# yunjinli/visual-slam

Hardware: AMD Instinct MI355X
Metric: stereo frames/sec, detect+describe (1500 feats) + stereo match, 752x480 (higher is better)
Workload: dtype u8/f32/f64; 1 GPU; synthetic 752x480 stereo, 1500 feats/frame (BASELINE configs[1]); independent streams per GPU (configs[3]); inputs_resident_in_hbm=True, distinct_stereo_pairs_per_gpu=1024, distinct_scenes_per_gpu=64, stereo_frames_per_pass_per_gpu=1024, hip_streams=2, stereo_frames_per_launch=512, num_features=1500, match=threshold 70, ratio 1.2, cross-check

## Files before the change

### visual-slam_amd/csrc/match.hip

```cpp
#include "vsl_common.h"

#ifndef VSL_MATCH_WAVES
#define VSL_MATCH_WAVES 8
#endif
#define KEY_SHIFT 22
#define KEY_INIT ((256u << KEY_SHIFT) | 0u)

__device__ __forceinline__ uint32_t umed3(uint32_t a, uint32_t b, uint32_t c) {
  uint32_t r;
  asm("v_med3_u32 %0, %1, %2, %3" : "=v"(r) : "v"(a), "v"(b), "v"(c));
  return r;
}

template <int WAVES>
__global__ __launch_bounds__(64 * WAVES) void hamming_best2_kernel(
    const uint64_t* __restrict__ desc, const int32_t* __restrict__ kp_count,
    const int32_t* __restrict__ pair_slots, uint32_t* __restrict__ best_key,
    uint32_t* __restrict__ second_key, int F) {
  const int pair = blockIdx.z, dir = blockIdx.y;
  const int slot_r = pair_slots[2 * pair + dir];
  const int slot_c = pair_slots[2 * pair + 1 - dir];
  const int n_r = kp_count[slot_r], n_c = kp_count[slot_c];
  const int row0 = blockIdx.x * 64;
  if (row0 >= n_r) return;
  const int lane = threadIdx.x & 63;
  const int wave = __builtin_amdgcn_readfirstlane(threadIdx.x >> 6);
  const int row = row0 + lane;

  uint32_t r[8];
  {
    const uint32_t* p = (const uint32_t*)(desc + ((size_t)slot_r * F + (row < n_r ? row : 0)) * 4);
#pragma unroll
    for (int k = 0; k < 8; k++) r[k] = p[k];
  }
  int chunk = (n_c + WAVES - 1) / WAVES;
  chunk = (chunk + 3) & ~3;
  const int c0 = wave * chunk;
  const int c1 = min(n_c, c0 + chunk);
  const uint32_t* __restrict__ cbase = (const uint32_t*)(desc + (size_t)slot_c * F * 4);

  uint32_t b = KEY_INIT, s = KEY_INIT;
  int j = c0;
  for (; j + 4 <= c1; j += 4) {
#pragma unroll
    for (int u = 0; u < 4; u++) {
      const uint32_t* __restrict__ c = cbase + (size_t)(j + u) * 8;
      uint32_t d = 0;
#pragma unroll
      for (int k = 0; k < 8; k++) d += __builtin_popcount(r[k] ^ c[k]);
      const uint32_t key = (d << KEY_SHIFT) | (uint32_t)(j + u);
      s = umed3(b, key, s);
      b = min(b, key);
    }
  }
  for (; j < c1; j++) {
    const uint32_t* __restrict__ c = cbase + (size_t)j * 8;
    uint32_t d = 0;
#pragma unroll
    for (int k = 0; k < 8; k++) d += __builtin_popcount(r[k] ^ c[k]);
    const uint32_t key = (d << KEY_SHIFT) | (uint32_t)j;
    s = umed3(b, key, s);
    b = min(b, key);
  }

  __shared__ uint32_t sb[WAVES][64], ss[WAVES][64];
  sb[wave][lane] = b;
  ss[wave][lane] = s;
  __syncthreads();
  if (wave == 0 && row < n_r) {
#pragma unroll
    for (int w = 1; w < WAVES; w++) {
      const uint32_t b2 = sb[w][lane], s2 = ss[w][lane];
      s = min(umed3(b, b2, s), s2);
      b = min(b, b2);
    }
    const size_t o = ((size_t)pair * 2 + dir) * F + row;
    best_key[o] = b;
    second_key[o] = s;
  }
}

typedef int v4i_t __attribute__((ext_vector_type(4)));
typedef int v16i_t __attribute__((ext_vector_type(16)));

#define MM_PAD_KEY (1023u << KEY_SHIFT)
#define MM_ROW 272

__device__ __forceinline__ v4i_t expand16(uint32_t bits16) {
  v4i_t o;
  o.x = (int)((((bits16 >> 0) & 15u) * 0x00204081u) & 0x01010101u);
  o.y = (int)((((bits16 >> 4) & 15u) * 0x00204081u) & 0x01010101u);
  o.z = (int)((((bits16 >> 8) & 15u) * 0x00204081u) & 0x01010101u);
  o.w = (int)((((bits16 >> 12) & 15u) * 0x00204081u) & 0x01010101u);
  return o;
}

#ifndef MM_WAVES
#define MM_WAVES 8
#endif
template <bool STAGGER>
__global__ __launch_bounds__(64 * MM_WAVES) void hamming_mfma_kernel(const uint64_t* __restrict__ desc,
                                                           const int32_t* __restrict__ kp_count,
                                                           const int32_t* __restrict__ pair_slots,
                                                           uint32_t* __restrict__ best_key,
                                                           uint32_t* __restrict__ second_key, int F) {
  __shared__ __align__(16) unsigned char tile[2][64 * MM_ROW];
  __shared__ __align__(16) uint32_t rowkey[3][64];
  const int pair = blockIdx.z, dir = blockIdx.y;
  const int slot_q = pair_slots[2 * pair + dir];
  const int slot_d = pair_slots[2 * pair + 1 - dir];
  const int n_q = kp_count[slot_q], n_d = kp_count[slot_d];
  const int q0 = blockIdx.x * (32 * MM_WAVES);
  if (q0 >= n_q) return;
  const int tid = threadIdx.x, lane = tid & 63, wave = tid >> 6;
  const int c = lane & 31, h = lane >> 5;
  const int qc = q0 + wave * 32 + c;
  const uint32_t* __restrict__ qd = (const uint32_t*)(desc + ((size_t)slot_q * F + (qc < n_q ? qc : 0)) * 4);
  const uint32_t* __restrict__ dbase = (const uint32_t*)(desc + (size_t)slot_d * F * 4);

  v4i_t bq[8];
  int pq = 0;
#pragma unroll
  for (int s = 0; s < 8; s++) {
    const uint32_t wq = qd[s];
    pq += __builtin_popcount(wq);
    const v4i_t e = expand16((wq >> (16 * h)) & 0xFFFFu);
    bq[s].x = (int)((uint32_t)e.x * 0xFEu + 0x01010101u);
    bq[s].y = (int)((uint32_t)e.y * 0xFEu + 0x01010101u);
    bq[s].z = (int)((uint32_t)e.z * 0xFEu + 0x01010101u);
    bq[s].w = (int)((uint32_t)e.w * 0xFEu + 0x01010101u);
  }

  constexpr int FILL_K = 64 * MM_WAVES >= 512 ? 1 : 512 / (64 * MM_WAVES);
  const bool filler = tid < 512;
  constexpr int FILL_ROWS = 64 / FILL_K;
  const int frow = tid >> 3, fword = tid & 7;
  auto load_words = [&](int st, uint32_t& w0, uint32_t& w1) {
    const int r0 = st * 64 + frow, r1 = r0 + FILL_ROWS;
    w0 = (filler && r0 < n_d) ? dbase[(size_t)r0 * 8 + fword] : 0u;
    w1 = (FILL_K > 1 && r1 < n_d) ? dbase[(size_t)r1 * 8 + fword] : 0u;
  };
  auto store_rows = [&](int buf, int st, uint32_t w0, uint32_t w1) {
    if (!filler) return;
#pragma unroll
    for (int k = 0; k < FILL_K; k++) {
      const uint32_t wd = k ? w1 : w0;
      const int lr = frow + FILL_ROWS * k;
      unsigned char* dst = &tile[buf][lr * MM_ROW + fword * 32];
      *(v4i_t*)dst = expand16(wd & 0xFFFFu);
      *(v4i_t*)(dst + 16) = expand16(wd >> 16);
      const int m = st * 64 + lr;
      if (fword == 0) rowkey[st % 3][lr] = m < n_d ? ((256u << KEY_SHIFT) | (uint32_t)m) : MM_PAD_KEY;
    }
  };
  const int n_st = (n_d + 63) / 64;
  uint32_t b = 0xFFFFFFFFu, sk = 0xFFFFFFFFu, bB = 0xFFFFFFFFu, skB = 0xFFFFFFFFu;
  {
    uint32_t w0, w1;
    load_words(0, w0, w1);
    store_rows(0, 0, w0, w1);
    __syncthreads();
  }
  v16i_t acc0, acc1;
  auto mfma_phase = [&](int buf) {
    acc0 = (v16i_t){0, 0, 0, 0, 0, 0, 0, 0, 0, 0, 0, 0, 0, 0, 0, 0};
    acc1 = (v16i_t){0, 0, 0, 0, 0, 0, 0, 0, 0, 0, 0, 0, 0, 0, 0, 0};
#pragma unroll
    for (int s = 0; s < 8; s++) {
      const v4i_t a0 = *(const v4i_t*)&tile[buf][c * MM_ROW + s * 32 + h * 16];
      const v4i_t a1 = *(const v4i_t*)&tile[buf][(c + 32) * MM_ROW + s * 32 + h * 16];
      acc0 = __builtin_amdgcn_mfma_i32_32x32x32_i8(a0, bq[s], acc0, 0, 0, 0);
      acc1 = __builtin_amdgcn_mfma_i32_32x32x32_i8(a1, bq[s], acc1, 0, 0, 0);
    }
  };
  auto key_phase = [&](int rk_slot) {
#pragma unroll
    for (int half = 0; half < 2; half++) {
#pragma unroll
      for (int g = 0; g < 4; g++) {
        const uint4 rk = *(const uint4*)&rowkey[rk_slot][32 * half + 8 * g + 4 * h];
        const uint32_t rks[4] = {rk.x, rk.y, rk.z, rk.w};
#pragma unroll
        for (int j = 0; j < 4; j++) {
          const int av = half ? acc1[4 * g + j] : acc0[4 * g + j];
          const uint32_t key = ((uint32_t)av << KEY_SHIFT) + rks[j];
          if (half) {
            skB = umed3(bB, key, skB);
            bB = min(bB, key);
          } else {
            sk = umed3(b, key, sk);
            b = min(b, key);
          }
        }
      }
    }
  };
  const bool late = STAGGER && wave >= MM_WAVES / 2;
  for (int st = 0; st < n_st; st++) {
    const int buf = st & 1;
    uint32_t n0 = 0, n1 = 0;
    if (st + 1 < n_st) load_words(st + 1, n0, n1);
    if (late) {
      if (st > 0) key_phase((st - 1) % 3);
      mfma_phase(buf);
    } else {
      mfma_phase(buf);
      key_phase(st % 3);
    }
    if (st + 1 < n_st) store_rows(buf ^ 1, st + 1, n0, n1);
    __syncthreads();
  }
  if (late && n_st > 0) key_phase((n_st - 1) % 3);
  sk = min(umed3(b, bB, sk), skB);
  b = min(b, bB);
  const uint32_t b2 = (uint32_t)__shfl_xor((int)b, 32), s2 = (uint32_t)__shfl_xor((int)sk, 32);
  sk = min(umed3(b, b2, sk), s2);
  b = min(b, b2);
  if (h == 0 && qc < n_q) {
    const uint32_t fix = (uint32_t)(pq - 256) << KEY_SHIFT;
    const size_t o = ((size_t)pair * 2 + dir) * F + qc;
    best_key[o] = (b >> KEY_SHIFT) >= 1023u ? KEY_INIT : b + fix;
    second_key[o] = (sk >> KEY_SHIFT) >= 1023u ? KEY_INIT : sk + fix;
  }
}

typedef int v8i_t __attribute__((ext_vector_type(8)));
typedef float v16f_t __attribute__((ext_vector_type(16)));
#define MX_ROW 144
#define MX_KEY_SCALE 2048.0f
#define MX_KEY_BIAS 512.0f
#define MX_PAD_KEY_F 4096.0f

__global__ __launch_bounds__(512) void match_select_kernel(const int32_t* __restrict__ kp_count, const int32_t* __restrict__ pair_slots,
                                                           const uint32_t* __restrict__ best_key,
                                                           const uint32_t* __restrict__ second_key, int F, int threshold,
                                                           double dist_2_best, int32_t* __restrict__ sel_list,
                                                           int32_t* __restrict__ sel_count) {
  __shared__ unsigned char flag[2048];
  __shared__ int sel_wave[8];
  const int pair = blockIdx.x, tid = threadIdx.x, lane = tid & 63, wave = tid >> 6;
  const int n_a = kp_count[pair_slots[2 * pair]], n_b = kp_count[pair_slots[2 * pair + 1]];
  const uint32_t* bk0 = best_key + ((size_t)pair * 2) * F;
  const uint32_t* sk0 = second_key + ((size_t)pair * 2) * F;
  for (int j = tid; j < 2048; j += 512) flag[j] = 0;
  __syncthreads();
  for (int i = tid; i < n_a; i += 512) {
    const uint32_t bk = bk0[i];
    const int d1 = (int)(bk >> KEY_SHIFT), d2 = (int)(sk0[i] >> KEY_SHIFT);
    if (n_b > 0 && d1 < threshold && !((double)d2 < (double)d1 * dist_2_best)) flag[bk & ((1u << KEY_SHIFT) - 1)] = 1;
  }
  __syncthreads();
  int cnt = 0;
#pragma unroll
  for (int u = 0; u < 4; u++) cnt += flag[tid * 4 + u];
  int incl = cnt;
#pragma unroll
  for (int d = 1; d < 64; d <<= 1) {
    const int o = __shfl_up(incl, d);
    if (lane >= d) incl += o;
  }
  if (lane == 63) sel_wave[wave] = incl;
  __syncthreads();
  int base = 0, total = 0;
#pragma unroll
  for (int w = 0; w < 8; w++) {
    if (w < wave) base += sel_wave[w];
    total += sel_wave[w];
  }
  int pos = base + incl - cnt;
  int32_t* out = sel_list + (size_t)pair * 2 * F;
#pragma unroll
  for (int u = 0; u < 4; u++)
    if (flag[tid * 4 + u]) out[pos++] = tid * 4 + u;
  if (tid == 0) sel_count[pair] = total;
}

#ifndef MX_WAVES_PER_EU
#define MX_WAVES_PER_EU 6
#endif
#ifndef MX_TIMING
#define MX_TIMING 0
#endif
#define MX_OCC __attribute__((amdgpu_waves_per_eu(MX_WAVES_PER_EU, MX_WAVES_PER_EU)))
#if MX_TIMING
__device__ long long mx_dbg[4 * 16];
__device__ long long mx_tl[4 * 3072];
extern "C" int vsl_mx_timing(long long* out) { return (int)hipMemcpyFromSymbol(out, HIP_SYMBOL(mx_dbg), sizeof(mx_dbg)); }
extern "C" int vsl_mx_timeline(long long* out) { return (int)hipMemcpyFromSymbol(out, HIP_SYMBOL(mx_tl), sizeof(mx_tl)); }
#endif
template <bool REVERSE>
__global__ __launch_bounds__(64 * MM_WAVES) MX_OCC void hamming_mx_kernel(const uint64_t* __restrict__ desc,
                                                                   const int32_t* __restrict__ kp_count,
                                                                   const int32_t* __restrict__ pair_slots,
                                                                   uint32_t* __restrict__ best_key,
                                                                   uint32_t* __restrict__ second_key, int F, int n_pairs,
                                                                   int blocks_per_pair, const int32_t* __restrict__ sel_list,
                                                                   const int32_t* __restrict__ sel_count, int both_dirs) {
  __shared__ __align__(16) unsigned char tile[2][64 * MX_ROW];
  __shared__ __align__(16) float rowkey[64];
  __shared__ uint32_t lut[256];
#if MX_TIMING
  const long long wEntry = wall_clock64();
#endif
  const int xj = (int)(blockIdx.x >> 3);
  const int pair = (xj / blocks_per_pair) * 8 + (int)(blockIdx.x & 7u);
  if (pair >= n_pairs) return;
  int blk = xj % blocks_per_pair;
  int dir = REVERSE ? 1 : 0;
  if (!REVERSE && both_dirs) {
    const int half = blocks_per_pair >> 1;
    dir = blk >= half ? 1 : 0;
    blk -= dir * half;
  }
  const int slot_q = pair_slots[2 * pair + dir];
  const int slot_d = pair_slots[2 * pair + 1 - dir];
  int n_q = kp_count[slot_q];
  const int n_d = kp_count[slot_d];
  const int q0 = blk * (32 * MM_WAVES);
  const int tid = threadIdx.x, lane = tid & 63, wave = tid >> 6;
  const int c = lane & 31, h = lane >> 5;
  const int32_t* __restrict__ sel = sel_list + (size_t)pair * 2 * F;
  if (REVERSE) n_q = sel_count[pair];
  if (q0 >= n_q) return;
  const int qc = q0 + wave * 32 + c;
  const int qrow = REVERSE ? sel[qc < n_q ? qc : 0] : (qc < n_q ? qc : 0);
  const uint32_t* __restrict__ qd = (const uint32_t*)(desc + ((size_t)slot_q * F + qrow) * 4);
  const uint32_t* __restrict__ dbase = (const uint32_t*)(desc + (size_t)slot_d * F * 4);
  if (tid < 256) {
    uint32_t x = (uint32_t)tid;
    x = (x | (x << 12)) & 0x000F000Fu;
    x = (x | (x << 6)) & 0x03030303u;
    x = (x | (x << 3)) & 0x11111111u;
    lut[tid] = x << 1;
  }
  __syncthreads();
  auto spread = [&](uint32_t w) -> v4i_t {
    v4i_t o;
    o.x = (int)lut[w & 255u];
    o.y = (int)lut[(w >> 8) & 255u];
    o.z = (int)lut[(w >> 16) & 255u];
    o.w = (int)lut[w >> 24];
    return o;
  };
  auto fp4_operand = [](v4i_t t) -> v8i_t { return __builtin_shufflevector(t, t, 0, 1, 2, 3, -1, -1, -1, -1); };
  v8i_t bq[4];
  int pq = 0;
#pragma unroll
  for (int s = 0; s < 4; s++) {
    const uint32_t w0 = qd[2 * s], w1 = qd[2 * s + 1];
    pq += __builtin_popcount(w0) + __builtin_popcount(w1);
    const v4i_t e = spread(h ? w1 : w0);
    bq[s] = fp4_operand((v4i_t){(int)(((uint32_t)e.x << 2) | 0x22222222u), (int)(((uint32_t)e.y << 2) | 0x22222222u),
                                (int)(((uint32_t)e.z << 2) | 0x22222222u), (int)(((uint32_t)e.w << 2) | 0x22222222u)});
  }
  const bool filler = tid < 512;
  const int frow = tid >> 3, fword = tid & 7;
  const int n_st = (n_d + 63) / 64;
  auto load_word = [&](int st) -> uint32_t {
    const int r0 = st * 64 + frow;
    return (filler && r0 < n_d) ? dbase[(size_t)r0 * 8 + fword] : 0u;
  };
  auto store_row = [&](int buf, int st, uint32_t wd) {
    if (!filler) return;
    *(v4i_t*)&tile[buf][frow * MX_ROW + fword * 16] = spread(wd);
    const int m = st * 64 + frow;
    if (fword == 0 && st == n_st - 1) rowkey[frow] = m < n_d ? (MX_KEY_BIAS + (float)m * (1.0f / MX_KEY_SCALE)) : MX_PAD_KEY_F;
  };
  uint32_t b = 0xFFFFFFFFu, sk = 0xFFFFFFFFu;
  auto fold3 = [](uint32_t& B, uint32_t& S, uint32_t k1, uint32_t k2, uint32_t k3) {
    const uint32_t lo = min(min(k1, k2), k3), mid = umed3(k1, k2, k3);
    S = umed3(B, lo, min(S, mid));
    B = min(B, lo);
  };
  auto tile_best2 = [&](uint32_t& L, uint32_t& M, const v16f_t& a) {
    uint32_t lo[5], mid[5];
#pragma unroll
    for (int t = 0; t < 5; t++) {
      const uint32_t k1 = __float_as_uint(a[3 * t]), k2 = __float_as_uint(a[3 * t + 1]), k3 = __float_as_uint(a[3 * t + 2]);
      lo[t] = min(min(k1, k2), k3);
      mid[t] = __float_as_uint(__builtin_amdgcn_fmed3f(a[3 * t], a[3 * t + 1], a[3 * t + 2]));
    }
    L = min(min(lo[0], lo[1]), lo[2]);
    M = umed3(lo[0], lo[1], lo[2]);
    fold3(L, M, lo[3], lo[4], __float_as_uint(a[15]));
    M = min(M, min(min(min(mid[0], mid[1]), mid[2]), min(mid[3], mid[4])));
  };
  v16f_t start;
#pragma unroll
  for (int i = 0; i < 16; i++) start[i] = MX_KEY_BIAS + (float)(8 * (i >> 2) + 4 * h + (i & 3)) * (1.0f / MX_KEY_SCALE);
  store_row(0, 0, load_word(0));
  __syncthreads();
  float tile_first = 0.0f;
  const bool idle = __builtin_amdgcn_readfirstlane(q0 + wave * 32) >= n_q;
#if MX_TIMING
  long long tA = 0, tB = 0, tC = 0;
  const long long w0 = wall_clock64();
#endif
  for (int st = 0; st < n_st; st++) {
#if MX_TIMING
    const long long s0 = __builtin_amdgcn_s_memtime();
#endif
    const int buf = st & 1;
    uint32_t nw = 0;
    if (st + 1 < n_st) nw = load_word(st + 1);
#define MX_QUAD(half, s) fp4_operand(*(const v4i_t*)&tile[buf][(c + 32 * (half)) * MX_ROW + (s) * 32 + h * 16])
    if (!idle)
#pragma unroll
    for (int half = 0; half < 2; half++) {
      v16f_t acc;
      if (st + 1 < n_st) {
        acc = __builtin_amdgcn_mfma_scale_f32_32x32x64_f8f6f4(MX_QUAD(half, 0), bq[0], start, 4, 4, 0, 127, 0, 127);
      } else {
#pragma unroll
        for (int g = 0; g < 4; g++) {
          const float4 r = *(const float4*)&rowkey[32 * half + 8 * g + 4 * h];
          acc[4 * g] = r.x, acc[4 * g + 1] = r.y, acc[4 * g + 2] = r.z, acc[4 * g + 3] = r.w;
        }
        acc = __builtin_amdgcn_mfma_scale_f32_32x32x64_f8f6f4(MX_QUAD(half, 0), bq[0], acc, 4, 4, 0, 127, 0, 127);
      }
#pragma unroll
      for (int s = 1; s < 4; s++) acc = __builtin_amdgcn_mfma_scale_f32_32x32x64_f8f6f4(MX_QUAD(half, s), bq[s], acc, 4, 4, 0, 127, 0, 127);
      uint32_t l, m;
      tile_best2(l, m, acc);
      if (st + 1 < n_st) {
        const float first = tile_first + (float)(32 * half) / MX_KEY_SCALE;
        l = __float_as_uint(__uint_as_float(l) + first), m = __float_as_uint(__uint_as_float(m) + first);
      }
      sk = umed3(b, l, min(sk, m));
      b = min(b, l);
    }
    tile_first += 64.0f / MX_KEY_SCALE;
#if MX_TIMING
    asm volatile("" ::"v"(b), "v"(sk));
    const long long s1 = __builtin_amdgcn_s_memtime();
#endif
    if (st + 1 < n_st) store_row(buf ^ 1, st + 1, nw);
#if MX_TIMING
    asm volatile("s_waitcnt lgkmcnt(0)");
    const long long s2 = __builtin_amdgcn_s_memtime();
#endif
    __syncthreads();
#if MX_TIMING
    const long long s3 = __builtin_amdgcn_s_memtime();
    tA += s1 - s0, tB += s2 - s1, tC += s3 - s2;
#endif
  }
#if MX_TIMING
  if (!REVERSE && tid == 0 && blockIdx.x < 3072) {
    mx_tl[4 * blockIdx.x] = wEntry, mx_tl[4 * blockIdx.x + 1] = w0, mx_tl[4 * blockIdx.x + 2] = wall_clock64();
    unsigned hw;
    asm volatile("s_getreg_b32 %0, hwreg(HW_REG_HW_ID)" : "=s"(hw));
    mx_tl[4 * blockIdx.x + 3] = hw;
  }
  if (!REVERSE && blockIdx.x == 1000 && lane == 0) {
    mx_dbg[4 * wave] = tA, mx_dbg[4 * wave + 1] = tB, mx_dbg[4 * wave + 2] = tC, mx_dbg[4 * wave + 3] = wall_clock64() - w0;
  }
#endif
  const uint32_t b2 = (uint32_t)__shfl_xor((int)b, 32), s2 = (uint32_t)__shfl_xor((int)sk, 32);
  sk = min(umed3(b, b2, sk), s2);
  b = min(b, b2);
  if (h == 0 && qc < n_q) {
    auto unpack = [&](uint32_t kb) -> uint32_t {
      if (kb >= __float_as_uint(MX_PAD_KEY_F)) return KEY_INIT;
      const int ki = (int)(__uint_as_float(kb) * MX_KEY_SCALE);
      return ((uint32_t)((ki >> 11) + pq - (int)MX_KEY_BIAS) << KEY_SHIFT) | (uint32_t)(ki & 2047);
    };
    const size_t o = ((size_t)pair * 2 + dir) * F + qrow;
    best_key[o] = unpack(b);
    second_key[o] = unpack(sk);
  }
}

__global__ __launch_bounds__(1024) void match_finalize_kernel(
    const int32_t* __restrict__ kp_count, const int32_t* __restrict__ pair_slots,
    const uint32_t* __restrict__ best_key, const uint32_t* __restrict__ second_key,
    int32_t* __restrict__ matches, int32_t* __restrict__ match_count, int F, int threshold,
    double dist_2_best) {
  const int pair = blockIdx.x;
  const int n_a = kp_count[pair_slots[2 * pair]];
  const int n_b = kp_count[pair_slots[2 * pair + 1]];
  const uint32_t* bk0 = best_key + ((size_t)pair * 2) * F;
  const uint32_t* sk0 = second_key + ((size_t)pair * 2) * F;
  const uint32_t* bk1 = bk0 + F;
  const uint32_t* sk1 = sk0 + F;
  __shared__ int wave_tot[16];
  __shared__ int base_s;
  if (threadIdx.x == 0) base_s = 0;
  __syncthreads();
  const int lane = threadIdx.x & 63, wave = threadIdx.x >> 6;
  for (int i0 = 0; i0 < n_a; i0 += 1024) {
    const int i = i0 + threadIdx.x;
    bool ok = false;
    int jbest = 0;
    if (i < n_a && n_b > 0) {
      const uint32_t b = bk0[i];
      const int d1 = (int)(b >> KEY_SHIFT);
      const int d2 = (int)(sk0[i] >> KEY_SHIFT);
      jbest = (int)(b & ((1u << KEY_SHIFT) - 1));
      if (d1 < threshold && !((double)d2 < (double)d1 * dist_2_best)) {
        const uint32_t rb = bk1[jbest];
        const int e1 = (int)(rb >> KEY_SHIFT);
        const int e2 = (int)(sk1[jbest] >> KEY_SHIFT);
        const int ri = (int)(rb & ((1u << KEY_SHIFT) - 1));
        ok = (e1 < threshold) && !((double)e2 < (double)e1 * dist_2_best) && ri == i;
      }
    }
    const unsigned long long m = __ballot(ok);
    const int within = __popcll(m & ((1ull << lane) - 1ull));
    if (lane == 0) wave_tot[wave] = __popcll(m);
    __syncthreads();
    int off = base_s;
    for (int w = 0; w < wave; w++) off += wave_tot[w];
    if (ok) {
      matches[((size_t)pair * F + off + within) * 2] = i;
      matches[((size_t)pair * F + off + within) * 2 + 1] = jbest;
    }
    __syncthreads();
    if (threadIdx.x == 0) {
      int t = 0;
      for (int w = 0; w < 16; w++) t += wave_tot[w];
      base_s += t;
    }
    __syncthreads();
  }
  if (threadIdx.x == 0) match_count[pair] = base_s;
}

int vsl_launch_match(vsl_ctx* ctx, vsl_frames* f, int n_pairs, int threshold, double dist_2_best, int db_bound) {
  if (n_pairs <= 0) return VSL_OK;
  constexpr int WAVES = VSL_MATCH_WAVES;
  {
    VslStage st(ctx, VSL_STAGE_MATCH);
    if (ctx->match_use_valu) {
      dim3 grid((f->F + 63) / 64, 2, n_pairs);
      hipLaunchKernelGGL(hamming_best2_kernel<WAVES>, grid, dim3(64 * WAVES), 0, ctx->stream, f->kp_desc,
                         f->kp_count, f->pair_slots, f->best_key, f->second_key, f->F);
    } else {
      dim3 grid((f->F + 32 * MM_WAVES - 1) / (32 * MM_WAVES), 2, n_pairs);
      if (db_bound <= 2048 && !ctx->match_use_i8) {
        const int bpp = (f->F + 32 * MM_WAVES - 1) / (32 * MM_WAVES);
        if (n_pairs < 8 && !ctx->match_two_pass) {
          const dim3 grid2((unsigned)(((n_pairs + 7) / 8) * 8 * 2 * bpp));
          hipLaunchKernelGGL(hamming_mx_kernel<false>, grid2, dim3(64 * MM_WAVES), 0, ctx->stream, f->kp_desc, f->kp_count,
                             f->pair_slots, f->best_key, f->second_key, f->F, n_pairs, 2 * bpp, (const int32_t*)f->matches,
                             (const int32_t*)f->match_count, 1);
        } else {
        const dim3 grid1((unsigned)(((n_pairs + 7) / 8) * 8 * bpp));
        hipLaunchKernelGGL(hamming_mx_kernel<false>, grid1, dim3(64 * MM_WAVES), 0, ctx->stream, f->kp_desc, f->kp_count,
                           f->pair_slots, f->best_key, f->second_key, f->F, n_pairs, bpp, (const int32_t*)f->matches,
                           (const int32_t*)f->match_count, 0);
        hipLaunchKernelGGL(match_select_kernel, dim3(n_pairs), dim3(512), 0, ctx->stream, f->kp_count, f->pair_slots, f->best_key,
                           f->second_key, f->F, threshold, dist_2_best, f->matches, f->match_count);
        hipLaunchKernelGGL(hamming_mx_kernel<true>, grid1, dim3(64 * MM_WAVES), 0, ctx->stream, f->kp_desc, f->kp_count,
                           f->pair_slots, f->best_key, f->second_key, f->F, n_pairs, bpp, (const int32_t*)f->matches,
                           (const int32_t*)f->match_count, 0);
        }
      } else if (ctx->match_no_stagger)
        hipLaunchKernelGGL(hamming_mfma_kernel<false>, grid, dim3(64 * MM_WAVES), 0, ctx->stream, f->kp_desc, f->kp_count,
                           f->pair_slots, f->best_key, f->second_key, f->F);
      else
        hipLaunchKernelGGL(hamming_mfma_kernel<true>, grid, dim3(64 * MM_WAVES), 0, ctx->stream, f->kp_desc, f->kp_count,
                           f->pair_slots, f->best_key, f->second_key, f->F);
    }
    VSL_CHECK_LAUNCH(ctx);
  }
  {
    VslStage st(ctx, VSL_STAGE_MATCH_FIN);
    hipLaunchKernelGGL(match_finalize_kernel, dim3(n_pairs), dim3(1024), 0, ctx->stream, f->kp_count,
                       f->pair_slots, f->best_key, f->second_key, f->matches, f->match_count, f->F, threshold,
                       dist_2_best);
    VSL_CHECK_LAUNCH(ctx);
  }
  return VSL_OK;
}

int vsl_set_pairs(vsl_ctx* ctx, vsl_frames* f, const int32_t* slot_pairs, int n_pairs) {
  const size_t n = 2 * (size_t)n_pairs;
  if (f->pair_cache.size() >= n && memcmp(f->pair_cache.data(), slot_pairs, n * sizeof(int32_t)) == 0) return VSL_OK;
  VSL_HIP(ctx, hipStreamSynchronize(ctx->stream));
  VSL_HIP(ctx, hipMemcpy(f->pair_slots, slot_pairs, n * sizeof(int32_t), hipMemcpyHostToDevice));
  f->pair_cache.assign(slot_pairs, slot_pairs + n);
  return VSL_OK;
}

extern "C" int vsl_frames_match(vsl_ctx* ctx, vsl_frames* f, const int32_t* slot_pairs, int n_pairs, int threshold,
                                double dist_2_best) {
  if (!ctx || !f || (n_pairs > 0 && !slot_pairs) || n_pairs < 0 || n_pairs > f->max_pairs)
    return vsl_fail(ctx, VSL_ERR_INVALID, "vsl_frames_match: bad arguments (n_pairs=%d, max_pairs=%d)", n_pairs, f ? f->max_pairs : -1);
  for (int i = 0; i < 2 * n_pairs; i++)
    if (slot_pairs[i] < 0 || slot_pairs[i] >= f->max_images)
      return vsl_fail(ctx, VSL_ERR_INVALID, "vsl_frames_match: slot %d out of range", slot_pairs[i]);
  if (n_pairs == 0) return VSL_OK;
  VSL_HIP(ctx, hipSetDevice(ctx->device));
  int rc = vsl_set_pairs(ctx, f, slot_pairs, n_pairs);
  if (rc) return rc;
  return vsl_launch_match(ctx, f, n_pairs, threshold, dist_2_best, f->F);
}

extern "C" int vsl_match_descriptors(vsl_ctx* ctx, const uint64_t* d1, int n1, const uint64_t* d2, int n2,
                                     int threshold, double dist_2_best, int32_t* pairs, int* n_out) {
  if (!ctx || !n_out || n1 < 0 || n2 < 0 || (n1 > 0 && !d1) || (n2 > 0 && !d2))
    return vsl_fail(ctx, VSL_ERR_INVALID, "vsl_match_descriptors: bad arguments");
  *n_out = 0;
  if (n1 == 0 || n2 == 0) return VSL_OK;
  if (n1 >= (1 << KEY_SHIFT) || n2 >= (1 << KEY_SHIFT))
    return vsl_fail(ctx, VSL_ERR_CAPACITY, "vsl_match_descriptors: at most %d descriptors per set", (1 << KEY_SHIFT) - 1);
  if (!pairs) return vsl_fail(ctx, VSL_ERR_INVALID, "vsl_match_descriptors: pairs is null");
  VSL_HIP(ctx, hipSetDevice(ctx->device));
  vsl_frames* f = nullptr;
  const int feat = n1 > n2 ? n1 : n2;
  int rc = vsl_ctx_scratch_frames(ctx, ctx->scratch ? ctx->scratch_w : 64, ctx->scratch ? ctx->scratch_h : 64,
                                  feat > (ctx->scratch ? ctx->scratch_feat : 0) ? feat : ctx->scratch_feat, &f);
  if (rc) return rc;
  const int32_t counts[2] = {n1, n2};
  const int32_t slots[2] = {0, 1};
  VSL_HIP(ctx, hipMemcpyAsync(f->kp_desc, d1, 32 * (size_t)n1, hipMemcpyHostToDevice, ctx->stream));
  VSL_HIP(ctx, hipMemcpyAsync(f->kp_desc + (size_t)f->F * 4, d2, 32 * (size_t)n2, hipMemcpyHostToDevice, ctx->stream));
  VSL_HIP(ctx, hipMemcpyAsync(f->kp_count, counts, sizeof(counts), hipMemcpyHostToDevice, ctx->stream));
  rc = vsl_set_pairs(ctx, f, slots, 1);
  if (rc) return rc;
  rc = vsl_launch_match(ctx, f, 1, threshold, dist_2_best, n1 > n2 ? n1 : n2);
  if (rc) return rc;
  return vsl_frames_download_matches(ctx, f, 0, n1 < n2 ? n1 : n2, pairs, n_out);
}
```

Measured before the change: 385,300 frames/s.

## Track only per-tile minimum in MX Hamming loop and recover second-best per class

Result: no change. 386,300 frames/s (median of 6 runs) (+0.3%).

```diff
diff --git a/visual-slam_amd/csrc/match.hip b/visual-slam_amd/csrc/match.hip
--- a/visual-slam_amd/csrc/match.hip
+++ b/visual-slam_amd/csrc/match.hip
@@ -231,23 +231,76 @@
 #define MX_KEY_BIAS 512.0f
 #define MX_PAD_KEY_F 4096.0f
 
-__global__ __launch_bounds__(512) void match_select_kernel(const int32_t* __restrict__ kp_count, const int32_t* __restrict__ pair_slots,
+__device__ __forceinline__ uint32_t class_second(bool need, int q, int m, const uint32_t* __restrict__ qbase,
+                                                 const uint32_t* __restrict__ dbase, int n_d) {
+  const int lane = threadIdx.x & 63, grp = lane >> 4, sub = lane & 15;
+  unsigned long long mask = __ballot(need && m < n_d);
+  uint32_t out = KEY_INIT;
+  while (mask) {
+    int src[4];
+#pragma unroll
+    for (int k = 0; k < 4; k++) {
+      src[k] = mask ? __ffsll((long long)mask) - 1 : -1;
+      mask &= mask - 1;
+    }
+    const int s = grp == 0 ? src[0] : grp == 1 ? src[1] : grp == 2 ? src[2] : src[3];
+    const int qi = __shfl(q, s < 0 ? 0 : s), mi = __shfl(m, s < 0 ? 0 : s);
+    const int r = (mi & ~31) | (mi & 4) | ((sub >> 2) << 3) | (sub & 3);
+    uint32_t key = KEY_INIT;
+    if (s >= 0 && r != mi && r < n_d) {
+      const uint4* qp = (const uint4*)(qbase + (size_t)qi * 8);
+      const uint4* dp = (const uint4*)(dbase + (size_t)r * 8);
+      const uint4 q0 = qp[0], q1 = qp[1], d0 = dp[0], d1 = dp[1];
+      const int d = __builtin_popcount(q0.x ^ d0.x) + __builtin_popcount(q0.y ^ d0.y) + __builtin_popcount(q0.z ^ d0.z) +
+                    __builtin_popcount(q0.w ^ d0.w) + __builtin_popcount(q1.x ^ d1.x) + __builtin_popcount(q1.y ^ d1.y) +
+                    __builtin_popcount(q1.z ^ d1.z) + __builtin_popcount(q1.w ^ d1.w);
+      key = ((uint32_t)d << KEY_SHIFT) | (uint32_t)r;
+    }
+#pragma unroll
+    for (int x = 1; x < 16; x <<= 1) key = min(key, (uint32_t)__shfl_xor((int)key, x));
+#pragma unroll
+    for (int k = 0; k < 4; k++) {
+      const uint32_t v = (uint32_t)__shfl((int)key, 16 * k);
+      if (lane == src[k]) out = v;
+    }
+  }
+  return out;
+}
+
+__global__ __launch_bounds__(512) void match_select_kernel(const uint64_t* __restrict__ desc, const int32_t* __restrict__ kp_count,
+                                                           const int32_t* __restrict__ pair_slots,
                                                            const uint32_t* __restrict__ best_key,
-                                                           const uint32_t* __restrict__ second_key, int F, int threshold,
+                                                           uint32_t* __restrict__ second_key, int F, int threshold,
                                                            double dist_2_best, int32_t* __restrict__ sel_list,
                                                            int32_t* __restrict__ sel_count) {
   __shared__ unsigned char flag[2048];
   __shared__ int sel_wave[8];
   const int pair = blockIdx.x, tid = threadIdx.x, lane = tid & 63, wave = tid >> 6;
-  const int n_a = kp_count[pair_slots[2 * pair]], n_b = kp_count[pair_slots[2 * pair + 1]];
+  const int slot_a = pair_slots[2 * pair], slot_b = pair_slots[2 * pair + 1];
+  const int n_a = kp_count[slot_a], n_b = kp_count[slot_b];
+  const uint32_t* __restrict__ da = (const uint32_t*)(desc + (size_t)slot_a * F * 4);
+  const uint32_t* __restrict__ db = (const uint32_t*)(desc + (size_t)slot_b * F * 4);
   const uint32_t* bk0 = best_key + ((size_t)pair * 2) * F;
-  const uint32_t* sk0 = second_key + ((size_t)pair * 2) * F;
+  uint32_t* sk0 = second_key + ((size_t)pair * 2) * F;
   for (int j = tid; j < 2048; j += 512) flag[j] = 0;
   __syncthreads();
-  for (int i = tid; i < n_a; i += 512) {
-    const uint32_t bk = bk0[i];
-    const int d1 = (int)(bk >> KEY_SHIFT), d2 = (int)(sk0[i] >> KEY_SHIFT);
-    if (n_b > 0 && d1 < threshold && !((double)d2 < (double)d1 * dist_2_best)) flag[bk & ((1u << KEY_SHIFT) - 1)] = 1;
+  for (int i0 = 0; i0 < n_a; i0 += 512) {
+    const int i = i0 + tid;
+    bool pass = false;
+    int d1 = 0, jbest = 0;
+    uint32_t sk = KEY_INIT;
+    if (i < n_a && n_b > 0) {
+      const uint32_t bk = bk0[i];
+      sk = sk0[i];
+      d1 = (int)(bk >> KEY_SHIFT), jbest = (int)(bk & ((1u << KEY_SHIFT) - 1));
+      pass = d1 < threshold && !((double)(int)(sk >> KEY_SHIFT) < (double)d1 * dist_2_best);
+    }
+    const uint32_t s2 = class_second(pass, i, jbest, da, db, n_b);
+    if (pass && s2 < sk) {
+      sk0[i] = s2;
+      pass = !((double)(int)(s2 >> KEY_SHIFT) < (double)d1 * dist_2_best);
+    }
+    if (pass) flag[jbest] = 1;
   }
   __syncthreads();
   int cnt = 0;
@@ -367,23 +420,13 @@
     if (fword == 0 && st == n_st - 1) rowkey[frow] = m < n_d ? (MX_KEY_BIAS + (float)m * (1.0f / MX_KEY_SCALE)) : MX_PAD_KEY_F;
   };
   uint32_t b = 0xFFFFFFFFu, sk = 0xFFFFFFFFu;
-  auto fold3 = [](uint32_t& B, uint32_t& S, uint32_t k1, uint32_t k2, uint32_t k3) {
-    const uint32_t lo = min(min(k1, k2), k3), mid = umed3(k1, k2, k3);
-    S = umed3(B, lo, min(S, mid));
-    B = min(B, lo);
-  };
-  auto tile_best2 = [&](uint32_t& L, uint32_t& M, const v16f_t& a) {
-    uint32_t lo[5], mid[5];
-#pragma unroll
-    for (int t = 0; t < 5; t++) {
-      const uint32_t k1 = __float_as_uint(a[3 * t]), k2 = __float_as_uint(a[3 * t + 1]), k3 = __float_as_uint(a[3 * t + 2]);
-      lo[t] = min(min(k1, k2), k3);
-      mid[t] = __float_as_uint(__builtin_amdgcn_fmed3f(a[3 * t], a[3 * t + 1], a[3 * t + 2]));
-    }
-    L = min(min(lo[0], lo[1]), lo[2]);
-    M = umed3(lo[0], lo[1], lo[2]);
-    fold3(L, M, lo[3], lo[4], __float_as_uint(a[15]));
-    M = min(M, min(min(min(mid[0], mid[1]), mid[2]), min(mid[3], mid[4])));
+  auto tile_min = [&](const v16f_t& a) -> uint32_t {
+    uint32_t lo[5];
+#pragma unroll
+    for (int t = 0; t < 5; t++)
+      lo[t] = min(min(__float_as_uint(a[3 * t]), __float_as_uint(a[3 * t + 1])), __float_as_uint(a[3 * t + 2]));
+    const uint32_t x = min(min(lo[0], lo[1]), lo[2]), y = min(min(lo[3], lo[4]), __float_as_uint(a[15]));
+    return min(x, y);
   };
   v16f_t start;
 #pragma unroll
@@ -420,13 +463,9 @@
       }
 #pragma unroll
       for (int s = 1; s < 4; s++) acc = __builtin_amdgcn_mfma_scale_f32_32x32x64_f8f6f4(MX_QUAD(half, s), bq[s], acc, 4, 4, 0, 127, 0, 127);
-      uint32_t l, m;
-      tile_best2(l, m, acc);
-      if (st + 1 < n_st) {
-        const float first = tile_first + (float)(32 * half) / MX_KEY_SCALE;
-        l = __float_as_uint(__uint_as_float(l) + first), m = __float_as_uint(__uint_as_float(m) + first);
-      }
-      sk = umed3(b, l, min(sk, m));
+      uint32_t l = tile_min(acc);
+      if (st + 1 < n_st) l = __float_as_uint(__uint_as_float(l) + (tile_first + (float)(32 * half) / MX_KEY_SCALE));
+      sk = umed3(b, sk, l);
       b = min(b, l);
     }
     tile_first += 64.0f / MX_KEY_SCALE;
@@ -472,13 +511,16 @@
 }
 
 __global__ __launch_bounds__(1024) void match_finalize_kernel(
-    const int32_t* __restrict__ kp_count, const int32_t* __restrict__ pair_slots,
+    const uint64_t* __restrict__ desc, const int32_t* __restrict__ kp_count, const int32_t* __restrict__ pair_slots,
     const uint32_t* __restrict__ best_key, const uint32_t* __restrict__ second_key,
     int32_t* __restrict__ matches, int32_t* __restrict__ match_count, int F, int threshold,
-    double dist_2_best) {
+    double dist_2_best, int refine_fwd, int refine_rev) {
   const int pair = blockIdx.x;
-  const int n_a = kp_count[pair_slots[2 * pair]];
-  const int n_b = kp_count[pair_slots[2 * pair + 1]];
+  const int slot_a = pair_slots[2 * pair], slot_b = pair_slots[2 * pair + 1];
+  const int n_a = kp_count[slot_a];
+  const int n_b = kp_count[slot_b];
+  const uint32_t* __restrict__ da = (const uint32_t*)(desc + (size_t)slot_a * F * 4);
+  const uint32_t* __restrict__ db = (const uint32_t*)(desc + (size_t)slot_b * F * 4);
   const uint32_t* bk0 = best_key + ((size_t)pair * 2) * F;
   const uint32_t* sk0 = second_key + ((size_t)pair * 2) * F;
   const uint32_t* bk1 = bk0 + F;
@@ -491,19 +533,29 @@
   for (int i0 = 0; i0 < n_a; i0 += 1024) {
     const int i = i0 + threadIdx.x;
     bool ok = false;
-    int jbest = 0;
+    int jbest = 0, d1 = 0, d2 = 0;
     if (i < n_a && n_b > 0) {
       const uint32_t b = bk0[i];
-      const int d1 = (int)(b >> KEY_SHIFT);
-      const int d2 = (int)(sk0[i] >> KEY_SHIFT);
+      d1 = (int)(b >> KEY_SHIFT);
+      d2 = (int)(sk0[i] >> KEY_SHIFT);
       jbest = (int)(b & ((1u << KEY_SHIFT) - 1));
-      if (d1 < threshold && !((double)d2 < (double)d1 * dist_2_best)) {
-        const uint32_t rb = bk1[jbest];
-        const int e1 = (int)(rb >> KEY_SHIFT);
-        const int e2 = (int)(sk1[jbest] >> KEY_SHIFT);
-        const int ri = (int)(rb & ((1u << KEY_SHIFT) - 1));
-        ok = (e1 < threshold) && !((double)e2 < (double)e1 * dist_2_best) && ri == i;
-      }
+      ok = d1 < threshold && !((double)d2 < (double)d1 * dist_2_best);
+    }
+    if (refine_fwd) {
+      d2 = min(d2, (int)(class_second(ok, i, jbest, da, db, n_b) >> KEY_SHIFT));
+      ok = ok && !((double)d2 < (double)d1 * dist_2_best);
+    }
+    int e1 = 0, e2 = 0, ri = 0;
+    if (ok) {
+      const uint32_t rb = bk1[jbest];
+      e1 = (int)(rb >> KEY_SHIFT);
+      e2 = (int)(sk1[jbest] >> KEY_SHIFT);
+      ri = (int)(rb & ((1u << KEY_SHIFT) - 1));
+      ok = (e1 < threshold) && !((double)e2 < (double)e1 * dist_2_best) && ri == i;
+    }
+    if (refine_rev) {
+      e2 = min(e2, (int)(class_second(ok, jbest, ri, db, da, n_a) >> KEY_SHIFT));
+      ok = ok && !((double)e2 < (double)e1 * dist_2_best);
     }
     const unsigned long long m = __ballot(ok);
     const int within = __popcll(m & ((1ull << lane) - 1ull));
@@ -529,6 +581,7 @@
 int vsl_launch_match(vsl_ctx* ctx, vsl_frames* f, int n_pairs, int threshold, double dist_2_best, int db_bound) {
   if (n_pairs <= 0) return VSL_OK;
   constexpr int WAVES = VSL_MATCH_WAVES;
+  int refine_fwd = 0, refine_rev = 0;
   {
     VslStage st(ctx, VSL_STAGE_MATCH);
     if (ctx->match_use_valu) {
@@ -544,16 +597,18 @@
           hipLaunchKernelGGL(hamming_mx_kernel<false>, grid2, dim3(64 * MM_WAVES), 0, ctx->stream, f->kp_desc, f->kp_count,
                              f->pair_slots, f->best_key, f->second_key, f->F, n_pairs, 2 * bpp, (const int32_t*)f->matches,
                              (const int32_t*)f->match_count, 1);
+          refine_fwd = refine_rev = 1;
         } else {
         const dim3 grid1((unsigned)(((n_pairs + 7) / 8) * 8 * bpp));
         hipLaunchKernelGGL(hamming_mx_kernel<false>, grid1, dim3(64 * MM_WAVES), 0, ctx->stream, f->kp_desc, f->kp_count,
                            f->pair_slots, f->best_key, f->second_key, f->F, n_pairs, bpp, (const int32_t*)f->matches,
                            (const int32_t*)f->match_count, 0);
-        hipLaunchKernelGGL(match_select_kernel, dim3(n_pairs), dim3(512), 0, ctx->stream, f->kp_count, f->pair_slots, f->best_key,
+        hipLaunchKernelGGL(match_select_kernel, dim3(n_pairs), dim3(512), 0, ctx->stream, f->kp_desc, f->kp_count, f->pair_slots, f->best_key,
                            f->second_key, f->F, threshold, dist_2_best, f->matches, f->match_count);
         hipLaunchKernelGGL(hamming_mx_kernel<true>, grid1, dim3(64 * MM_WAVES), 0, ctx->stream, f->kp_desc, f->kp_count,
                            f->pair_slots, f->best_key, f->second_key, f->F, n_pairs, bpp, (const int32_t*)f->matches,
                            (const int32_t*)f->match_count, 0);
+        refine_rev = 1;
         }
       } else if (ctx->match_no_stagger)
         hipLaunchKernelGGL(hamming_mfma_kernel<false>, grid, dim3(64 * MM_WAVES), 0, ctx->stream, f->kp_desc, f->kp_count,
@@ -566,9 +621,9 @@
   }
   {
     VslStage st(ctx, VSL_STAGE_MATCH_FIN);
-    hipLaunchKernelGGL(match_finalize_kernel, dim3(n_pairs), dim3(1024), 0, ctx->stream, f->kp_count,
+    hipLaunchKernelGGL(match_finalize_kernel, dim3(n_pairs), dim3(1024), 0, ctx->stream, f->kp_desc, f->kp_count,
                        f->pair_slots, f->best_key, f->second_key, f->matches, f->match_count, f->F, threshold,
-                       dist_2_best);
+                       dist_2_best, refine_fwd, refine_rev);
     VSL_CHECK_LAUNCH(ctx);
   }
   return VSL_OK;
```
